# knights-lab/UTree

Hardware: AMD Instinct MI355X
Metric: reads classified/sec, 8 GB L2 CTR, 150 bp reads (higher is better)
Workload: dtype u64; 1 GPU; configs[1]: 1.22e+09-node synthetic L2 CTR (k=32, 21844 labels, image 40.8 GiB, fine_bits=8), 1152000000 x 150 bp reads per GPU (72 steps x 16000000-read batches, 41 distinct batches resident in HBM), RC=0

## Files before the change

utree_amd/csrc/dev_image.c:

```c
#define _FILE_OFFSET_BITS 64
#define _GNU_SOURCE
#define __HIP_PLATFORM_AMD__ 1
#include <hip/hip_runtime_api.h>
#include <fcntl.h>
#include <math.h>
#include <stddef.h>
#include <stdio.h>
#include <stdlib.h>
#include <string.h>
#include <unistd.h>
#include "ctr_host.h"
#include "dev_image.h"

#define HIPCHK(x) do { hipError_t e_ = (x); if (e_ != hipSuccess) { utree_dev_set_hip_error((int)e_, #x); rc = e_ == hipErrorOutOfMemory ? UTREE_E_NOMEM : UTREE_E_HIP; goto fail; } } while (0)
#define KCHK(x) do { int e_ = (x); if (e_ != 0) { utree_dev_set_hip_error(e_, #x); rc = e_ == (int)hipErrorOutOfMemory ? UTREE_E_NOMEM : UTREE_E_HIP; goto fail; } } while (0)

static __thread char g_hip_msg[256];
void utree_dev_set_hip_error(int err, const char *what) {
    snprintf(g_hip_msg, sizeof g_hip_msg, "%s (%d) in %s", hipGetErrorString((hipError_t)err), err, what);
    if (getenv("UTREE_DEBUG")) fprintf(stderr, "[utree_amd] HIP error: %s\n", g_hip_msg);
}
const char *utree_last_hip_error(void) { return g_hip_msg; }
void utree_set_error_text(const char *msg) { snprintf(g_hip_msg, sizeof g_hip_msg, "%s", msg); }

// ... 788 lines not shown
        d->last_long = w.long_blocks != 0; d->last_mid = 0; d->last_rc = do_rc; d->last_short_cap = w.short_cap;
        d->last_lanes = utk_lanes_segs(&d->kimg, max_len); d->last_mixed = mixed; d->last_pieces = w.long_blocks != 0;
        if (e0 && !w.long_blocks) HIPCHK(hipEventRecord(e0, st));
        if (!mixed) KCHK(utk_classify_lanes(&d->kimg, d_bases, d_off, d_len, n_reads, max_len, do_rc, d_out, &w, d->n_cu, st));
        else KCHK(utk_classify_lanes_mixed(&d->kimg, d_bases, d_off, d_len, n_reads, max_len, do_rc, d_out, &w, d->n_cu, st));
        if (w.long_blocks) {
            if (e0) HIPCHK(hipEventRecord(e0, st));
            HIPCHK(hipMemsetAsync(w.ltab_rank, 0xFF, (size_t)w.n_long_cap * UTREE_LONG_SLOTS * 4, st));
            HIPCHK(hipMemsetAsync(w.ltab_cnt, 0, (size_t)w.n_long_cap * UTREE_LONG_SLOTS * 4, st));
            HIPCHK(hipMemsetAsync(w.lflag, 0, (size_t)w.n_long_cap * 4, st));
            KCHK(utk_classify_long_pieces(&d->kimg, d_bases, d_off, d_len, do_rc, d_out, &w, d->n_cu, st));
            utk_workspace wl = w;
            wl.long_list = w.long_left;
            wl.long_blocks = w.long_blocks >= 8 ? w.long_blocks / 8 : 1;
            KCHK(utk_classify_long(&d->kimg, d_bases, d_off, d_len, do_rc, d_out, &wl, d->n_cu, st));
            if (e0) { HIPCHK(hipEventRecord(e1, st)); d->recorded[tslot] = 1; }
        }
        KCHK(utk_classify_listed(&d->kimg, d_bases, d_off, d_len, n_reads, max_len, do_rc, d_out, &w, d->n_cu, st));
        if (e0 && !w.long_blocks) { HIPCHK(hipEventRecord(e1, st)); d->recorded[tslot] = 1; }
    } else {
        const int dominant = w.long_blocks ? 2 : (w.mid_reads ? 1 : 0);
        d->last_long = dominant == 2; d->last_mid = dominant == 1; d->last_rc = do_rc; d->last_short_cap = w.short_cap;
        d->last_lanes = 0; d->last_mixed = 0; d->last_pieces = 0;
        if (w.mid_reads) KCHK(utk_route(d_len, n_reads, do_rc, &w, st));
        if (e0 && dominant == 0) HIPCHK(hipEventRecord(e0, st));
        KCHK(utk_classify_short(&d->kimg, d_bases, d_off, d_len, n_reads, do_rc, d_out, &w, d->n_cu, st));
        if (e0 && dominant == 0) { HIPCHK(hipEventRecord(e1, st)); d->recorded[tslot] = 1; }
        if (w.mid_reads) {
            if (e0 && dominant == 1) HIPCHK(hipEventRecord(e0, st));
            KCHK(utk_classify_mid(&d->kimg, d_bases, d_off, d_len, n_reads, do_rc, d_out, &w, d->n_cu, st));
            if (e0 && dominant == 1) { HIPCHK(hipEventRecord(e1, st)); d->recorded[tslot] = 1; }
        }
        if (w.long_blocks) {
            if (e0) HIPCHK(hipEventRecord(e0, st));
            KCHK(utk_classify_long(&d->kimg, d_bases, d_off, d_len, do_rc, d_out, &w, d->n_cu, st));
            if (e0) { HIPCHK(hipEventRecord(e1, st)); d->recorded[tslot] = 1; }
        }
    }
    if (rd && (rc = utree_redist_add_pending(rd, &d->kimg, d_out, &w, n_reads, d->n_cu, st))) goto fail;
    KCHK(utk_vote(&d->kimg, d_out, &w, n_reads, st));
    if (ring_post(d, &w, lanes ? n_reads : 0, st)) { (void)hipGetLastError(); }
    { ring_lock(d); const unsigned long long pe = d->dev_error; ring_unlock(d);
      if (pe) { rc = UTREE_E_DEVICE; snprintf(g_hip_msg, sizeof g_hip_msg, "an earlier batch's kernels reported error %llu: utree_classify_poll returns (and clears) it", pe); } }
#ifdef UTREE_LANES_TIMERS
    { extern void utk_lanes_phase_dump(void); static int lcalls; if (++lcalls == 6) utk_lanes_phase_dump(); }
#endif
#ifdef UTREE_PHASE_TIMERS
    { extern void utk_phase_dump(void); static int calls; if (++calls == 12) utk_phase_dump(); }
#endif
fail:
    return rc;
}

int utree_lookup_words(utree_dev *d, const uint64_t *d_hi, const uint64_t *d_lo, uint64_t n, uint32_t *d_ix, void *stream) {
    int rc = UTREE_OK;
    if (!d || !d_lo || !d_ix) return UTREE_E_ARG;
    if (d->hdr.W == 16 && !d_hi) return UTREE_E_ARG;
    HIPCHK(hipSetDevice(d->device));
    KCHK(utk_lookup(&d->kimg, d_hi, d_lo, n, d_ix, (hipStream_t)stream));
fail:
    return rc;
}

const char *utree_classify_kernel_name(const utree_dev *dc) {
    if (!dc) return "";
    utree_dev *d = (utree_dev *)dc;
    if (d->last_lanes && d->last_pieces) {
        snprintf(d->kernel_sig, sizeof d->kernel_sig, "classify_lanes_k<%u, %u, 16, %s, 2, %u, %s>", d->hdr.W, d->hdr.I, d->kimg.irr_n ? "true" : "false", d->hdr.bucket_words / 8,
                 utk_lanes_both_strands(&d->kimg, d->last_rc) ? "true" : "false");
        return d->kernel_sig;
    }
    if (d->last_lanes && d->last_mixed) {
        snprintf(d->kernel_sig, sizeof d->kernel_sig, "classify_lanes_mixed_k<%u, %u, %s, %u, %s>", d->hdr.W, d->hdr.I, d->kimg.irr_n ? "true" : "false",
                 d->hdr.bucket_words / 8, utk_lanes_both_strands(&d->kimg, d->last_rc) ? "true" : "false");
        return d->kernel_sig;
    }
    if (d->last_lanes) {
        snprintf(d->kernel_sig, sizeof d->kernel_sig, "classify_lanes_k<%u, %u, 1, %s, 0, %u, %s>", d->hdr.W, d->hdr.I, d->kimg.irr_n ? "true" : "false",
                 d->hdr.bucket_words / 8, utk_lanes_both_strands(&d->kimg, d->last_rc) ? "true" : "false");
        return d->kernel_sig;
    }
    return d->last_long ? utk_classify_long_name(&d->kimg, d->kernel_sig, sizeof d->kernel_sig)
                        : utk_classify_short_name(&d->kimg, d->last_short_cap ? d->last_short_cap : UTREE_SHORT_CAP, d->last_mid, d->last_rc,
                                                  d->kernel_sig, sizeof d->kernel_sig);
}

int utree_model_counts(utree_dev *d, const uint8_t *d_bases, const uint64_t *d_off, const uint32_t *d_len, uint32_t n_reads,
                       int do_rc, uint64_t *h_counts5, void *stream) {
    int rc = UTREE_OK;
    unsigned long long *dc = NULL;
    if (!d || !d_bases || !d_off || !d_len || !h_counts5) return UTREE_E_ARG;
    HIPCHK(hipSetDevice(d->device));
    HIPCHK(hipMalloc((void **)&dc, 64));
    HIPCHK(hipMemsetAsync(dc, 0, 64, (hipStream_t)stream));
    KCHK(utk_model_counts(&d->kimg, d_bases, d_off, d_len, n_reads, do_rc, dc, stream));
    HIPCHK(hipMemcpyAsync(h_counts5, dc, 40, hipMemcpyDeviceToHost, (hipStream_t)stream));
    HIPCHK(hipStreamSynchronize((hipStream_t)stream));
fail:
    if (dc) hipFree(dc);
    return rc;
}

int utree_classify_kernel_time(utree_dev *d, int reset, double *ms_total, uint64_t *launches) {
    int rc = UTREE_OK;
    if (!d) return UTREE_E_ARG;
    HIPCHK(hipSetDevice(d->device));
// ... 20 lines not shown
```

utree_amd/csrc/kernels.hip:

```cpp
#include <hip/hip_runtime.h>
#include <stdint.h>
#include <stdio.h>
#include <string.h>
#include "device_common.hpp"
#include "wave_common.hpp"

using namespace utk;

namespace {

#ifdef UTREE_PHASE_TIMERS
__device__ unsigned long long g_phase[16];
struct PhaseT { unsigned long long t, acc[12]; };
#define PH_DECL PhaseT ph_; ph_.t = __builtin_readcyclecounter(); for (int q_ = 0; q_ < 12; ++q_) ph_.acc[q_] = 0;
#define TICKP(ph, i) do { const unsigned long long n_ = __builtin_readcyclecounter(); (ph).acc[i] += n_ - (ph).t; (ph).t = n_; } while (0)
#define TICK(i) TICKP(ph_, i)
#define PH_ARG , PhaseT &ph_
#define PH_PASS , ph_
#define PH_WAITVM asm volatile("s_waitcnt vmcnt(0)" ::: "memory")
#else
#define PH_DECL
#define TICK(i)
#define PH_ARG
#define PH_PASS
// ... 618 lines not shown
__device__ __forceinline__ uint32_t cut_of(uint32_t x) {
    uint32_t c = x - x / 4;
    c += (x >> 1) >= c;
    return c;
}

__device__ __forceinline__ void label16(const char *s, uint32_t p, uint64_t &x, uint64_t &y) {
    typedef unsigned long long u64x2 __attribute__((ext_vector_type(2), aligned(1)));
    const u64x2 v = *(const u64x2 *)(s + p);
    x = v.x; y = v.y;
}

__device__ __forceinline__ uint64_t stop_flags(uint64_t x1, uint64_t x2) {
    const uint64_t semi = x1 ^ 0x3B3B3B3B3B3B3B3Bull, d = x1 ^ x2;
    uint64_t m = (((x1 - 0x0101010101010101ull) & ~x1) | ((semi - 0x0101010101010101ull) & ~semi)) & 0x8080808080808080ull;
    m |= (((d & 0x7F7F7F7F7F7F7F7Full) + 0x7F7F7F7F7F7F7F7Full) | d) & 0x8080808080808080ull;
    return m;
}

__device__ __forceinline__ void pair_scan(const char *s1, const char *s2, uint32_t start, uint32_t &td, uint32_t &a, uint32_t &b, uint32_t &before) {
    uint32_t base = start, prevlast = start ? (uint32_t)(uint8_t)s1[start - 1] : 0u;
    for (;;) {
        uint64_t x1, y1, x2, y2;
        label16(s1, base, x1, y1); label16(s2, base, x2, y2);
        uint64_t m = stop_flags(x1, x2);
        if (!m) { prevlast = (uint32_t)(x1 >> 56); base += 8; x1 = y1; x2 = y2; m = stop_flags(x1, x2); }
        if (m) {
            const uint32_t idx = (uint32_t)(__builtin_ctzll(m) >> 3);
            td = base + idx;
            a = (uint32_t)(x1 >> (8 * idx)) & 0xFFu; b = (uint32_t)(x2 >> (8 * idx)) & 0xFFu;
            before = idx ? ((uint32_t)(x1 >> (8 * idx - 8)) & 0xFFu) : prevlast;
            return;
        }
        prevlast = (uint32_t)(x1 >> 56); base += 8;
    }
}

struct VRec { uint64_t w[4]; };
__device__ __forceinline__ VRec vrec(const uint64_t *vt, uint32_t rank) {
    typedef unsigned long long u64x2 __attribute__((ext_vector_type(2)));
    const u64x2 *p = (const u64x2 *)(vt + (size_t)rank * 4);
    const u64x2 a = p[0], b = p[1];
    VRec v; v.w[0] = a.x; v.w[1] = a.y; v.w[2] = b.x; v.w[3] = b.y;
    return v;
}
__device__ __forceinline__ uint32_t v_pid(const VRec &v, uint32_t t) { return (uint32_t)((t < 4 ? v.w[0] : v.w[1]) >> (16u * (t & 3u))) & 0xFFFFu; }
__device__ __forceinline__ uint32_t v_end(const VRec &v, uint32_t t) { return (uint32_t)(v.w[2] >> (8u * t)) & 0xFFu; }
__device__ __forceinline__ bool v_exists(const VRec &v, uint32_t t) { return ((uint32_t)v.w[3] >> t) & 1u; }
__device__ __forceinline__ bool v_more(const VRec &v, uint32_t t) { return ((uint32_t)v.w[3] >> (8u + t)) & 1u; }
__device__ __forceinline__ bool v_us(const VRec &v, uint32_t t) { return ((uint32_t)v.w[3] >> (16u + t)) & 1u; }
__device__ __forceinline__ uint32_t v_len(const VRec &v) { return (uint32_t)(v.w[3] >> 32) & 0xFFu; }
__device__ __forceinline__ uint32_t v_ix(const VRec &v) { return (uint32_t)(v.w[3] >> 48); }

__device__ __forceinline__ void vote_table(const utk_image &im, utree_result *out_r, const uint64_t *T, uint32_t F, uint32_t uix) {
    const uint64_t *vt = im.vote_tab;
    const char *blob = im.label_blob;
    const uint32_t *loff = im.label_off;
    constexpr uint32_t NONE = 0xFFFFFFFFu;
    uint32_t cutoff = cut_of(F);
    uint32_t st = 0, ed = uix, dv = NONE, t = 0, orun = F, sl, ol;
    uint32_t ix_last, n_last, len_last;
    for (;;) {
        const uint64_t t_st = T[st];
        VRec pv = vrec(vt, (uint32_t)t_st);
        const uint64_t t_ed = ed - 1u == st ? t_st : T[ed - 1u];
        const VRec lv = ed - 1u == st ? pv : vrec(vt, (uint32_t)t_ed);
        {
            const uint64_t d0 = pv.w[0] ^ lv.w[0], d1 = pv.w[1] ^ lv.w[1];
            const uint32_t same = d0 ? (uint32_t)__builtin_ctzll(d0) >> 4 : 4u + (d1 ? (uint32_t)__builtin_ctzll(d1) >> 4 : 4u);
            const uint32_t both = ((uint32_t)(pv.w[3] & lv.w[3]) >> 8) & 0xFFu;
            const uint32_t semis = (uint32_t)__builtin_ctz(~both);
            const uint32_t L = same < semis ? same : semis;
            if (L > t) { dv = v_end(pv, L - 1u); t = L; }
        }
        uint32_t run = (uint32_t)(t_st >> 32), td = dv, c1 = run, rp = (uint32_t)t_st;
        bool td_is_end = false;
        bool stopped = false;
        for (uint32_t z = st + 1; z < ed; ++z) {
            const bool is_last = z == ed - 1u;
            const uint64_t tz = is_last ? t_ed : T[z];
            const uint32_t nz = (uint32_t)(tz >> 32), rc = (uint32_t)tz;
            const VRec cv = is_last ? lv : vrec(vt, rc);
            bool aside = false, stop = false;
            if (t >= 8u || !v_exists(pv, t) || (dv == NONE && v_end(pv, 0) == 0u && !v_more(pv, 0))) aside = true;
            else {
                uint32_t a, b, before;
                bool known = true;
                if (v_exists(cv, t) && v_pid(cv, t) == v_pid(pv, t)) {
                    td = v_end(pv, t); td_is_end = true;
                    a = v_more(pv, t) ? ';' : 0u; b = v_more(cv, t) ? ';' : 0u; before = v_us(pv, t) ? '_' : 'x';
                } else if (v_us(pv, t) || !v_exists(cv, t)) {
                    pair_scan(blob + loff[rp], blob + loff[rc], dv + 1u, td, a, b, before);
                    td_is_end = td == v_end(pv, t);
                } else { a = 'a'; b = 'b'; before = 'x'; known = false; }
                if (a == b) run += nz;
                else if ((!a && b == ';') || ((a == ';' || !a) && before == '_')) aside = true;
                else if (run >= cutoff) {
                    ed = z; stop = true;
                    if (!known) {
                        pair_scan(blob + loff[rp], blob + loff[rc], dv + 1u, td, a, b, before);
                        td_is_end = td == v_end(pv, t);
                    }
                } else { run = nz; st = z; }
            }
            if (aside) {
                run = nz; st = z;
                orun -= c1;
                cutoff = cut_of(orun);
            }
            if (stop) { stopped = true; break; }
            pv = cv; c1 = nz; rp = rc;
        }
        ix_last = stopped ? v_ix(pv) : v_ix(lv);
        n_last = stopped ? c1 : (uint32_t)(t_ed >> 32);
        len_last = stopped ? v_len(pv) : v_len(lv);
        sl = run; ol = orun;
        if (run < cutoff) break;
        if (st + 1 >= ed) {
            if (n_last >= cutoff) dv = 0xFFFFFFFEu;
            break;
        }
        orun = run; cutoff = cut_of(run);
        if (td != dv) { dv = td; if (td_is_end) ++t; }
    }
    int32_t cut;
    if (dv == NONE) cut = -1;
    else if (dv == 0xFFFFFFFEu) cut = -2;
    else cut = (int32_t)(dv < len_last ? dv : len_last);
    store_result(out_r, ix_last, cut, F, uix, sl, ol);
}

__global__ __launch_bounds__(256) void vote_table_k(utk_image im, utree_result *__restrict__ out, utk_workspace ws, uint32_t n_reads) {
    __shared__ uint32_t s_n[2][4];
    __shared__ uint16_t s_who[256];
    const uint32_t tid = threadIdx.x, wv = tid >> 6, lane = tid & 63u;
    const uint32_t r0 = blockIdx.x * blockDim.x + tid;
    uint32_t cls = 2;
    if (r0 < n_reads) {
        const uint32_t *res = (const uint32_t *)&out[r0];
        const int32_t cut = (int32_t)res[1];
        if (cut == RANK_PENDING) {
            uint32_t *o = (uint32_t *)&out[r0];
            o[0] = im.rank2ix[res[0]]; o[1] = (uint32_t)-2;
        } else if (cut == CUT_PENDING) cls = res[3] == 2u ? 0u : 1u;
    }
    const uint64_t m0 = __builtin_amdgcn_ballot_w64(cls == 0u), m1 = __builtin_amdgcn_ballot_w64(cls == 1u);
    s_who[tid] = 0xFFFFu;
    if (lane == 0) { s_n[0][wv] = (uint32_t)__popcll(m0); s_n[1][wv] = (uint32_t)__popcll(m1); }
    __syncthreads();
    if (cls < 2u) {
        uint32_t before = 0;
        for (uint32_t w = 0; w < wv; ++w) before += s_n[cls][w];
        before += (uint32_t)__popcll((cls ? m1 : m0) & ((1ull << lane) - 1ull));
        s_who[cls ? 255u - before : before] = (uint16_t)tid;
    }
    __syncthreads();
    const uint32_t who = s_who[tid];
    if (who == 0xFFFFu) return;
    const uint32_t r = blockIdx.x * blockDim.x + who;
    const uint32_t *res = (const uint32_t *)&out[r];
    vote_table(im, &out[r], ws.tally + ((uint64_t)res[4] | ((uint64_t)res[5] << 32)), res[2], res[3]);
}

__global__ __launch_bounds__(256) void vote_k(utk_image im, utree_result *__restrict__ out, utk_workspace ws, uint32_t n_reads) {
    const uint32_t r = blockIdx.x * blockDim.x + threadIdx.x;
    if (r >= n_reads) return;
    const uint32_t *res = (const uint32_t *)&out[r];
    if ((int32_t)res[1] == RANK_PENDING) {
        uint32_t *o = (uint32_t *)&out[r];
        o[0] = im.rank2ix[res[0]]; o[1] = (uint32_t)-2;
        return;
    }
    if ((int32_t)res[1] != CUT_PENDING) return;
    const uint32_t F = res[2], uix = res[3];
    const uint64_t *T = ws.tally + ((uint64_t)res[4] | ((uint64_t)res[5] << 32));
    const char *blob = im.label_blob;
    const uint32_t *loff = im.label_off;
    uint32_t cutoff = cut_of(F);
    uint32_t st = 0, ed = uix, dv = 0xFFFFFFFFu, orun = F, sl, ol;
    for (;;) {
        const uint64_t t_st = T[st];
        {
            const char *sa = blob + loff[(uint32_t)t_st], *sz = blob + loff[(uint32_t)T[ed - 1]];
            uint32_t base = dv + (dv == 0xFFFFFFFFu), q = 0xFFFFFFFFu;
            bool first = dv != 0xFFFFFFFFu;
            for (;;) {
                uint64_t a[2], b[2];
                label16(sa, base, a[0], a[1]); label16(sz, base, b[0], b[1]);
                bool stop = false;
#pragma unroll
                for (int h = 0; h < 2; ++h) {
                    const uint64_t x = a[h], d = a[h] ^ b[h], sx = a[h] ^ 0x3B3B3B3B3B3B3B3Bull;
                    uint64_t end = ((x - 0x0101010101010101ull) & ~x) & 0x8080808080808080ull;
                    end |= (((d & 0x7F7F7F7F7F7F7F7Full) + 0x7F7F7F7F7F7F7F7Full) | d) & 0x8080808080808080ull;
                    uint64_t semi = ~(((sx & 0x7F7F7F7F7F7F7F7Full) + 0x7F7F7F7F7F7F7F7Full) | sx) & 0x8080808080808080ull;
                    if (h == 0 && first) { end &= ~0xFFull; semi &= ~0xFFull; }
                    if (end) semi &= (end & (0ull - end)) - 1ull;
                    if (semi) q = base + 8u * (uint32_t)h + ((63u - (uint32_t)__builtin_clzll(semi)) >> 3);
                    if (end) { stop = true; break; }
                }
                if (stop) break;
                base += 16; first = false;
            }
            if (q != 0xFFFFFFFFu) dv = q;
        }
        uint32_t run = (uint32_t)(t_st >> 32), td = dv;
        const char *s1 = blob + loff[(uint32_t)t_st];
        uint32_t c1 = run;
        const uint32_t probe = dv + (dv == 0xFFFFFFFFu);
        const bool skip0 = dv != 0xFFFFFFFFu;
        uint64_t x1_first, y1_first;
        label16(s1, probe, x1_first, y1_first);
        for (uint32_t z = st + 1; z < ed; ++z) {
            const uint64_t tz = T[z];
// ... 146 lines not shown
    });
}

int utk_route(const uint32_t *d_len, uint32_t n_reads, int do_rc, const utk_workspace *ws, void *stream) {
    if (!n_reads) return 0;
    route_k<<<dim3((n_reads + 255) / 256), dim3(256), 0, (hipStream_t)stream>>>(d_len, n_reads, do_rc, *ws);
    return (int)hipGetLastError();
}

int utk_classify_mid(const utk_image *im, const uint8_t *d_bases, const uint64_t *d_off, const uint32_t *d_len,
                     uint32_t n_reads, int do_rc, utree_result *d_out, const utk_workspace *ws, int n_cu, void *stream) {
    if (!n_reads) return 0;
    uint32_t blocks = (n_reads + WAVES_PER_BLOCK - 1) / WAVES_PER_BLOCK;
    uint32_t cap = (uint32_t)n_cu * 5u;
    if (blocks > cap) blocks = cap;
    return dispatch_img_all(im, [&](auto w, auto i, auto exc, auto offt) {
        classify_short_k<decltype(w)::value, decltype(i)::value, decltype(exc)::value, decltype(offt), MID_CAP, true>
            <<<dim3(blocks), dim3(256), 0, (hipStream_t)stream>>>(*im, d_bases, d_off, d_len, n_reads, do_rc, d_out, *ws);
    });
}

int utk_classify_listed(const utk_image *im, const uint8_t *d_bases, const uint64_t *d_off, const uint32_t *d_len,
                        uint32_t n_reads, uint32_t max_len, int do_rc, utree_result *d_out, const utk_workspace *ws, int n_cu, void *stream) {
    if (!n_reads) return 0;
    uint32_t blocks = (n_reads + WAVES_PER_BLOCK - 1) / WAVES_PER_BLOCK;
    uint32_t cap = (uint32_t)n_cu * 2u;
    if (blocks > cap) blocks = cap;
    const uint64_t total = do_rc ? 2ull * max_len + 1 : max_len;
    return dispatch_img(im, [&](auto w, auto i, auto exc, auto offt) {
        if (total > SHORT2_CAP)
            classify_short_k<decltype(w)::value, decltype(i)::value, decltype(exc)::value, decltype(offt), MID_CAP, true>
                <<<dim3(blocks), dim3(256), 0, (hipStream_t)stream>>>(*im, d_bases, d_off, d_len, n_reads, do_rc, d_out, *ws);
        else if (do_rc || total > SHORT_CAP)
            classify_short_k<decltype(w)::value, decltype(i)::value, decltype(exc)::value, decltype(offt), SHORT2_CAP, true>
                <<<dim3(blocks), dim3(256), 0, (hipStream_t)stream>>>(*im, d_bases, d_off, d_len, n_reads, do_rc, d_out, *ws);
        else
            classify_short_k<decltype(w)::value, decltype(i)::value, decltype(exc)::value, decltype(offt), SHORT_CAP, true, 0>
                <<<dim3(blocks), dim3(256), 0, (hipStream_t)stream>>>(*im, d_bases, d_off, d_len, n_reads, do_rc, d_out, *ws);
    });
}

int utk_classify_long(const utk_image *im, const uint8_t *d_bases, const uint64_t *d_off, const uint32_t *d_len,
                      int do_rc, utree_result *d_out, const utk_workspace *ws, int n_cu, void *stream) {
    (void)n_cu;
    if (!ws->long_blocks) return 0;
    return dispatch_img_all(im, [&](auto w, auto i, auto exc, auto offt) {
        classify_long_k<decltype(w)::value, decltype(i)::value, decltype(exc)::value, decltype(offt)>
            <<<dim3(ws->long_blocks), dim3(LONG_THREADS), 0, (hipStream_t)stream>>>(*im, d_bases, d_off, d_len, do_rc, d_out, *ws);
    });
}

int utk_vote(const utk_image *im, utree_result *d_out, const utk_workspace *ws, uint32_t n_reads, void *stream) {
    if (!n_reads) return 0;
    if (im->vote_tab) vote_table_k<<<dim3((n_reads + 255) / 256), dim3(256), 0, (hipStream_t)stream>>>(*im, d_out, *ws, n_reads);
    else vote_k<<<dim3((n_reads + 255) / 256), dim3(256), 0, (hipStream_t)stream>>>(*im, d_out, *ws, n_reads);
    return (int)hipGetLastError();
}

int utk_lookup(const utk_image *im, const uint64_t *d_hi, const uint64_t *d_lo, uint64_t n, uint32_t *d_ix, void *stream) {
    if (!n) return 0;
    uint64_t blocks = (n + 255) / 256;
    if (blocks > 8192) blocks = 8192;
    return dispatch_img_all(im, [&](auto w, auto i, auto exc, auto offt) {
        lookup_k<decltype(w)::value, decltype(i)::value, decltype(exc)::value, decltype(offt)>
            <<<dim3((unsigned)blocks), dim3(256), 0, (hipStream_t)stream>>>(*im, d_hi, d_lo, n, d_ix);
    });
}

#ifdef UTREE_PHASE_TIMERS
void utk_phase_dump(void) {
    unsigned long long h[16];
    static const char *nm[12] = {"grab", "next read's len/off + fetch issue", "minimizers", "round: address (LDS chain) + load issue", "round: wait for the bucket",
                                 "round: scan", "round: hit compaction", "stage next read (waits for its bytes)", "tally + result", "after windows", "", ""};
    if (hipDeviceSynchronize() != hipSuccess || hipMemcpyFromSymbol(h, HIP_SYMBOL(g_phase), sizeof h) != hipSuccess) return;
    unsigned long long tot = 0;
    for (int q = 0; q < 12; ++q) tot += h[q];
    fprintf(stderr, "[phase timers] %llu waves, %.3g cycles per wave\n", h[12], h[12] ? (double)tot / h[12] : 0.0);
    for (int q = 0; q < 10; ++q) fprintf(stderr, "  %-45s %5.1f %%\n", nm[q], tot ? 100.0 * h[q] / tot : 0.0);
    memset(h, 0, sizeof h);
    (void)hipMemcpyToSymbol(HIP_SYMBOL(g_phase), h, sizeof h);
}
#endif

int utk_model_counts(const utk_image *im, const uint8_t *d_bases, const uint64_t *d_off, const uint32_t *d_len, uint32_t n_reads,
                     int do_rc, unsigned long long *d_counts, void *stream) {
    if (!n_reads) return 0;
    uint32_t blocks = (n_reads + 3) / 4;
    if (blocks > 4096) blocks = 4096;
    return dispatch_wi(im->W, im->I, [&](auto w, auto i) {
        model_k<decltype(w)::value, decltype(i)::value><<<dim3(blocks), dim3(256), 0, (hipStream_t)stream>>>(*im, d_bases, d_off, d_len, n_reads,
                                                                                                      do_rc, d_counts);
    });
}

static const char *kernel_signature(char *buf, size_t cap, const char *name, const utk_image *im, int slice, int listed, int rcmode) {
    const bool exc = (im->flags & (UTREE_F_IRREGULAR | UTREE_F_GENERIC)) != 0, o64 = (im->flags & UTREE_F_OFF64) != 0;
    if (slice) snprintf(buf, cap, "%s<%u, %u, %s, %s, %d, %s, %d>", name, im->W, im->I, exc ? "true" : "false", o64 ? "unsigned long" : "unsigned int",
                        slice, listed ? "true" : "false", rcmode);
    else snprintf(buf, cap, "%s<%u, %u, %s, %s>", name, im->W, im->I, exc ? "true" : "false", o64 ? "unsigned long" : "unsigned int");
    return buf;
}
const char *utk_classify_short_name(const utk_image *im, uint32_t short_cap, int mid, int do_rc, char *buf, size_t cap) {
    if (mid) return kernel_signature(buf, cap, "classify_short_k", im, MID_CAP, 1, 2);
    if (short_cap == UTREE_SHORT2_CAP) return kernel_signature(buf, cap, "classify_short_k", im, SHORT2_CAP, 0, 2);
    return kernel_signature(buf, cap, "classify_short_k", im, SHORT_CAP, 0, do_rc ? 1 : 0);
}
const char *utk_classify_long_name(const utk_image *im, char *buf, size_t cap) { return kernel_signature(buf, cap, "classify_long_k", im, 0, 0, 0); }
// ... 3 lines not shown
```

utree_amd/csrc/utree_internal.h:

```cpp
#ifndef UTREE_INTERNAL_H
#define UTREE_INTERNAL_H
#include <stddef.h>
#include <stdint.h>
#include <stdlib.h>
#include <time.h>
#include "../../include/utree_amd.h"

#ifdef __cplusplus
extern "C" {
#endif

#define UTREE_NUMBINS ((1u << 24) + 1u)
#define UTREE_INVALID 0xFFFFFFFFu
#define UTREE_IMG_MAGIC 0x31474d4945525455ull
#define UTREE_IMG_HEADER_BYTES 4096u
#define UTREE_IMG_VERSION 14u
#define UTREE_REGION_NB_BITS 25
#define UTREE_REGION_SUB_BITS 9
#define UTREE_REGION_BASE_SHIFT (UTREE_REGION_NB_BITS + UTREE_REGION_SUB_BITS)
#define UTREE_MIN_MARGIN(W_) ((W_) == 16 ? 2u : 0u)
#define UTREE_TALLY_CHUNK 8192u
#define UTREE_CUR_LONG 32
#define UTREE_CUR_MID 16
#define UTREE_CUR_WORK 48
// ... 78 lines not shown
                  const uint64_t *d_regions, const uint64_t *h_regions, uint64_t n_buckets, uint32_t bucket_words, uint64_t *d_table, uint64_t *d_mrecs,
                  uint32_t *d_irreg, unsigned long long *d_overflow, uint64_t *n_min, int *views, void *stream);
int utk_build_direct(uint32_t I, int off64, int generic, const void *d_coarse, const uint64_t *d_recs, uint64_t n_nodes, uint64_t c0, uint64_t m,
                     const uint32_t *d_irreg, uint64_t n_irregular, void *d_table, void *stream);
int utk_compact_overflow(uint32_t W, uint32_t I, uint64_t *d_table, uint64_t n_buckets, uint32_t bucket_words, uint64_t *d_mrecs, uint64_t *n_kept, int *chains, void *stream);
int utk_compress_chunk(uint32_t W, uint32_t I, const void *d_in, uint64_t first, uint64_t count, unsigned long long *d_first,
                       void *d_out, void *stream);
int utk_fill_recs_pad(uint64_t *d_recs_end, uint32_t words, void *stream);

typedef struct {
    unsigned long long *cursors;
    uint64_t *tally;
    uint64_t tally_cap;
    uint32_t *long_list;
    uint32_t *mid_list;
    uint32_t *hist;
    uint32_t *touch;
    uint32_t long_blocks, mid_reads;
    uint32_t short_cap;
    uint32_t mid_limit;
    uint64_t *pieces;
    uint32_t *ltab_rank, *ltab_cnt;
    uint32_t *lflag;
    uint32_t *long_left;
    uint32_t n_long_cap;
    uint64_t n_pieces_cap;
    uint32_t *cls_list;
    uint32_t cls_stride;
    uint64_t ltally_base;
} utk_workspace;

int utk_classify_short(const utk_image *im, const uint8_t *d_bases, const uint64_t *d_off, const uint32_t *d_len,
                       uint32_t n_reads, int do_rc, utree_result *d_out, const utk_workspace *ws, int n_cu,
                       void *stream);
int utk_lanes_ok(const utk_image *im, uint32_t max_len, int do_rc);
int utk_lanes_segs(const utk_image *im, uint32_t max_len);
int utk_lanes_image_ok(const utk_image *im);
int utk_lanes_both_strands(const utk_image *im, int do_rc);
int utk_classify_long_pieces(const utk_image *im, const uint8_t *d_bases, const uint64_t *d_off, const uint32_t *d_len, int do_rc,
                             utree_result *d_out, const utk_workspace *ws, int n_cu, void *stream);
int utk_classify_lanes(const utk_image *im, const uint8_t *d_bases, const uint64_t *d_off, const uint32_t *d_len, uint32_t n_reads,
                       uint32_t max_len, int do_rc, utree_result *d_out, const utk_workspace *ws, int n_cu, void *stream);
int utk_classify_lanes_mixed(const utk_image *im, const uint8_t *d_bases, const uint64_t *d_off, const uint32_t *d_len, uint32_t n_reads,
                             uint32_t max_len, int do_rc, utree_result *d_out, const utk_workspace *ws, int n_cu, void *stream);
uint32_t utk_lanes_max_len(const utk_image *im);
int utk_route(const uint32_t *d_len, uint32_t n_reads, int do_rc, const utk_workspace *ws, void *stream);
int utk_classify_mid(const utk_image *im, const uint8_t *d_bases, const uint64_t *d_off, const uint32_t *d_len,
                     uint32_t n_reads, int do_rc, utree_result *d_out, const utk_workspace *ws, int n_cu, void *stream);
int utk_classify_listed(const utk_image *im, const uint8_t *d_bases, const uint64_t *d_off, const uint32_t *d_len,
                        uint32_t n_reads, uint32_t max_len, int do_rc, utree_result *d_out, const utk_workspace *ws, int n_cu, void *stream);
int utk_classify_long(const utk_image *im, const uint8_t *d_bases, const uint64_t *d_off, const uint32_t *d_len,
                      int do_rc, utree_result *d_out, const utk_workspace *ws, int n_cu, void *stream);
int utk_vote(const utk_image *im, utree_result *d_out, const utk_workspace *ws, uint32_t n_reads, void *stream);
int utk_lookup(const utk_image *im, const uint64_t *d_hi, const uint64_t *d_lo, uint64_t n, uint32_t *d_ix,
               void *stream);
typedef struct {
    unsigned long long *cursors;
    uint32_t *nh;
    uint64_t *hoff;
    uint32_t *hits;
    uint64_t hits_cap;
    uint32_t *lvl[3];
    uint32_t nlvl[3];
    uint32_t *hist;
    uint32_t hist_waves;
    uint32_t *state;
    uint32_t state_cap;
    uint32_t step;
    uint32_t slack, tolerance;
} utk_rank_ws;

int utk_rank_hits(const utk_image *im, const uint8_t *d_bases, const uint64_t *d_off, const uint32_t *d_len,
                  uint32_t n_reads, int do_rc, const utk_rank_ws *ws, int n_cu, void *stream);
int utk_rank_levels(const utk_rank_ws *ws, uint32_t n_reads, void *stream);
int utk_rank_vote(const utk_image *im, utree_result *d_out, uint32_t n_reads, const utk_rank_ws *ws, int n_cu,
                  void *stream);
int utk_rank_state(uint32_t n_reads, const utk_rank_ws *ws, void *stream);

const char *utk_classify_short_name(const utk_image *im, uint32_t short_cap, int mid, int do_rc, char *buf, size_t cap);
const char *utk_classify_long_name(const utk_image *im, char *buf, size_t cap);
int utk_model_counts(const utk_image *im, const uint8_t *d_bases, const uint64_t *d_off, const uint32_t *d_len, uint32_t n_reads,
                     int do_rc, unsigned long long *d_counts, void *stream);

static inline double now_s(void) { struct timespec ts; clock_gettime(CLOCK_MONOTONIC, &ts); return (double)ts.tv_sec + 1e-9 * (double)ts.tv_nsec; }
static inline int timing_on(void) { return getenv("UTREE_TIMING") != NULL || getenv("UTREE_DEBUG") != NULL; }
int utree_pread_team(int fd, void *dst, size_t bytes, uint64_t off, int max_threads);

#ifdef __cplusplus
}
#endif
#endif
```

utree_amd/lib.py:

```python
from __future__ import annotations

import ctypes as C
import os

_HERE = os.path.dirname(os.path.abspath(__file__))
SO_PATH = os.environ.get("UTREE_AMD_SO") or os.path.join(_HERE, "libutree_amd.so")
CLI_PATH = os.path.join(_HERE, "xtree-searchGG")
COMPRESS_CLI_PATH = os.path.join(_HERE, "xtree-compress")
RANK_CLI_PATH = os.path.join(_HERE, "xtree-search")
BUILD_GG_CLI_PATH = os.path.join(_HERE, "utree-buildGG")
BUILD_CLI_PATH = os.path.join(_HERE, "utree-build")
_LIB = None

OK, E_IO, E_FORMAT, E_UNSUPPORTED, E_NOMEM, E_HIP, E_ARG, E_NOLABELS, E_FASTA, E_RCCL, E_BUILD, E_DEVICE, E_PROFILE, E_COVERAGE, E_PAIRS = range(15)
BUILD_E_MAP_EMPTY, BUILD_E_MAP, BUILD_E_FASTA, BUILD_E_NO_KMERS, BUILD_E_NAME = range(1, 6)
FINE_AUTO = -1
FANOUT_NONE, FANOUT_BROADCAST, FANOUT_UPLOAD = range(3)
REPLICATE_FN = C.CFUNCTYPE(C.c_int, C.c_void_p, C.c_void_p, C.POINTER(C.c_int), C.c_int, C.POINTER(C.c_void_p))
UPLOAD_FN = C.CFUNCTYPE(C.c_int, C.c_void_p, C.c_int, C.c_int, C.POINTER(C.c_void_p))
INPUT_REFERENCE, INPUT_FASTQ, INPUT_FASTA_MULTILINE, INPUT_AUTO = range(4)


class CtrInfo(C.Structure):
    _fields_ = [("W", C.c_uint32), ("I", C.c_uint32), ("k", C.c_uint32), ("SZ", C.c_uint32), ("n_nodes", C.c_uint64),
# ... 112 lines not shown
    "utree_rank_search_file": (C.c_int, [C.c_void_p, C.c_void_p, C.c_char_p, C.c_char_p, C.c_int, C.POINTER(RankParams),
                                         C.c_int, C.POINTER(SearchStats)]),
    "utree_reads_frame": (C.c_int, [C.c_void_p, C.c_size_t, C.c_int, C.c_int, C.c_size_t, C.c_void_p, C.c_void_p, C.c_void_p,
                                    C.c_void_p, C.POINTER(C.c_size_t), C.POINTER(C.c_size_t), C.POINTER(FastaError)]),
    "utree_search_file_opts": (C.c_int, [C.c_void_p, C.POINTER(C.c_void_p), C.c_int, C.c_char_p, C.c_char_p, C.c_int, C.c_int,
                                         C.c_int, C.POINTER(SearchStats)]),
    "utree_rank_search_file_opts": (C.c_int, [C.c_void_p, C.c_void_p, C.c_char_p, C.c_char_p, C.c_int, C.POINTER(RankParams),
                                              C.c_int, C.c_int, C.POINTER(SearchStats)]),
    "utree_build_file": (C.c_int, [C.c_char_p, C.c_char_p, C.c_char_p, C.c_uint32, C.c_uint32, C.c_int, C.c_int, C.c_int,
                                   C.POINTER(BuildStats)]),
    "utree_search_prepare": (C.c_int, [C.c_void_p, C.POINTER(C.c_void_p), C.c_int, C.c_int]),
    "utree_search_file": (C.c_int, [C.c_void_p, C.POINTER(C.c_void_p), C.c_int, C.c_char_p, C.c_char_p, C.c_int, C.c_int,
                                    C.POINTER(SearchStats)]),
    "utree_profile_create": (C.c_int, [C.c_void_p, C.c_uint32, C.POINTER(C.c_void_p)]),
    "utree_profile_add": (C.c_int, [C.c_void_p, C.c_void_p, C.c_uint32, C.c_void_p]),
    "utree_profile_reset": (C.c_int, [C.c_void_p]),
    "utree_profile_max_entries": (C.c_size_t, [C.c_void_p]),
    "utree_profile_read": (C.c_int, [C.c_void_p, C.c_void_p, C.c_size_t, C.POINTER(C.c_size_t), C.POINTER(C.c_uint64),
                                     C.POINTER(C.c_uint64)]),
    "utree_profile_free": (None, [C.c_void_p]),
    "utree_profile_write": (C.c_int, [C.c_void_p, C.c_void_p, C.c_size_t, C.c_uint64, C.c_char_p]),
    "utree_search_file_profile": (C.c_int, [C.c_void_p, C.POINTER(C.c_void_p), C.c_int, C.c_char_p, C.c_char_p, C.c_int, C.c_int,
                                            C.c_int, C.c_char_p, C.POINTER(SearchStats)]),
    "utree_coverage_bytes": (C.c_size_t, [C.c_void_p]),
    "utree_coverage_create": (C.c_int, [C.c_void_p, C.c_void_p, C.c_void_p, C.c_void_p, C.POINTER(C.c_void_p)]),
    "utree_coverage_add": (C.c_int, [C.c_void_p, C.c_void_p, C.c_void_p, C.c_void_p, C.c_uint32, C.c_int, C.c_void_p]),
    "utree_coverage_reset": (C.c_int, [C.c_void_p]),
    "utree_coverage_merge": (C.c_int, [C.c_void_p, C.c_void_p]),
    "utree_coverage_read": (C.c_int, [C.c_void_p, C.c_void_p, C.c_size_t, C.POINTER(C.c_size_t), C.POINTER(C.c_uint64),
                                      C.POINTER(C.c_uint64)]),
    "utree_coverage_free": (None, [C.c_void_p]),
    "utree_coverage_write": (C.c_int, [C.c_void_p, C.c_void_p, C.c_size_t, C.c_uint64, C.c_char_p]),
    "utree_search_file_coverage": (C.c_int, [C.c_void_p, C.POINTER(C.c_void_p), C.c_int, C.c_char_p, C.c_char_p, C.c_int, C.c_int,
                                             C.c_int, C.c_char_p, C.c_char_p, C.POINTER(SearchStats)]),
    "utree_redist_create": (C.c_int, [C.c_void_p, C.c_uint32, C.POINTER(C.c_void_p)]),
    "utree_redist_reset": (C.c_int, [C.c_void_p]),
    "utree_redist_free": (None, [C.c_void_p]),
    "utree_redist_classify_batch": (C.c_int, [C.c_void_p, C.c_void_p, C.c_void_p, C.c_void_p, C.c_void_p, C.c_uint32, C.c_uint64,
                                              C.c_uint32, C.c_int, C.c_void_p, C.c_void_p, C.c_size_t, C.c_void_p]),
    "utree_redist_read": (C.c_int, [C.c_void_p, C.c_void_p, C.c_size_t, C.c_void_p, C.c_size_t, C.POINTER(C.c_size_t), C.POINTER(C.c_size_t),
                                    C.POINTER(C.c_uint64), C.POINTER(C.c_uint64)]),
    "utree_redist_merge": (C.c_int, [C.c_void_p, C.c_void_p]),
    "utree_redist_solve": (C.c_int, [C.c_void_p, C.c_uint32, C.c_void_p, C.c_size_t, C.POINTER(C.c_size_t), C.POINTER(C.c_uint32),
                                     C.POINTER(C.c_uint64)]),
    "utree_redist_write": (C.c_int, [C.c_void_p, C.c_void_p, C.c_size_t, C.c_uint64, C.c_uint64, C.c_uint32, C.c_char_p]),
    "utree_search_file_redistribute": (C.c_int, [C.c_void_p, C.POINTER(C.c_void_p), C.c_int, C.c_char_p, C.c_char_p, C.c_int, C.c_char_p, C.c_int,
                                                 C.c_int, C.c_int, C.c_char_p, C.c_char_p, C.c_char_p, C.c_uint32, C.POINTER(SearchStats)]),
    "utree_pairs_join": (C.c_int, [C.c_void_p, C.c_void_p, C.c_void_p, C.c_void_p, C.c_void_p, C.c_void_p, C.c_void_p, C.c_uint32, C.c_void_p,
                                   C.c_uint64, C.c_void_p, C.c_void_p, C.c_void_p, C.c_void_p]),
    "utree_search_pairs_file": (C.c_int, [C.c_void_p, C.POINTER(C.c_void_p), C.c_int, C.c_char_p, C.c_char_p, C.c_char_p, C.c_int, C.c_int,
                                          C.c_int, C.c_char_p, C.c_char_p, C.POINTER(SearchStats)]),
    "utree_rank_search_file_profile": (C.c_int, [C.c_void_p, C.c_void_p, C.c_char_p, C.c_char_p, C.c_int, C.POINTER(RankParams),
                                                 C.c_int, C.c_int, C.c_char_p, C.POINTER(SearchStats)]),
}


def kernel_source_sha256() -> str:
    import hashlib
    h = hashlib.sha256()
    for f in ("kernels.hip", "lanes_kernel.hip", "lanes_core.hpp", "lanes_part.hip", "wave_common.hpp", "device_common.hpp", "utree_internal.h", "Makefile"):
        with open(os.path.join(_HERE, "csrc", f), "rb") as fh:
            h.update(f.encode() + b"\0" + fh.read() + b"\0")
    return h.hexdigest()


class UtreeError(RuntimeError):
    def __init__(self, code, what=""):
        self.code = code
        msg = load().utree_strerror(code).decode() if _LIB is not None else str(code)
        if _LIB is not None and code in (4, 5, 11, 12, 13, 14):
            hip = (_LIB.utree_last_hip_error() or b"").decode(errors="replace")
            if hip:
                msg += " [" + hip + "]"
        super().__init__("%s: %s (code %d)" % (what, msg, code))


def load():
    global _LIB
    if _LIB is None:
        if not os.path.exists(SO_PATH):
            raise ImportError("utree_amd: %s is missing -- build it with `make -C utree_amd/csrc` "
                              "(or __graft_entry__.build()); there is no CPU fallback" % SO_PATH)
        try:
            import torch
        except ImportError:
            pass
        L = C.CDLL(SO_PATH, mode=C.RTLD_GLOBAL)
        for name, (res, args) in SYMBOLS.items():
            f = getattr(L, name)
            f.restype = res
            f.argtypes = args
        _LIB = L
    return _LIB


def check(code, what=""):
    if code != OK:
        raise UtreeError(code, what)
```

Before: 2.358 billion reads/s.

## Bin vote-table reads by label count per 2048-read tile and specialize small cases

The vote_table kernel now processes 2048-read tiles per block. It classifies pending reads into buckets by distinct-label count (2, 3, 4, other), compacts them through shared memory so each wavefront runs reads of the same size class, and calls vote_table instances templated on N with the loop unrolled and, for two labels, records preloaded. The aim is to cut wavefront divergence and loop overhead in the LCA vote. It also adds a host-side utree_vote_lists test entry point, which is unrelated to speed. The risks are more shared-memory and register pressure and fewer blocks in flight.

```diff
diff --git a/utree_amd/csrc/dev_image.c b/utree_amd/csrc/dev_image.c
--- a/utree_amd/csrc/dev_image.c
+++ b/utree_amd/csrc/dev_image.c
@@ -864,6 +864,65 @@
     return rc;
 }
 
+static int vote_ent_cmp(const void *a, const void *b) {
+    const uint64_t x = *(const uint64_t *)a, y = *(const uint64_t *)b;
+    return (uint32_t)x < (uint32_t)y ? -1 : (uint32_t)x > (uint32_t)y;
+}
+int utree_vote_lists(utree_dev *d, const uint32_t *h_ix, const uint32_t *h_cnt, const uint32_t *h_first, uint32_t n_reads, utree_result *h_out) {
+    int rc = UTREE_OK;
+    if (!d || !h_first || !h_out || (h_first[n_reads] && (!h_ix || !h_cnt))) return UTREE_E_ARG;
+    if (!n_reads) return UTREE_OK;
+    const uint32_t n_labels = d->hdr.n_labels, total = h_first[n_reads];
+    uint32_t *ix2rank = (uint32_t *)calloc((size_t)n_labels + 1, 4), *r2i = (uint32_t *)malloc(((size_t)n_labels + 1) * 4);
+    uint64_t *tally = (uint64_t *)malloc(((size_t)total + 1) * 8);
+    uint32_t *rec = (uint32_t *)calloc((size_t)n_reads, sizeof(utree_result));
+    void *d_out = NULL, *d_tally = NULL;
+    if (!ix2rank || !r2i || !tally || !rec) { rc = UTREE_E_NOMEM; goto fail; }
+    HIPCHK(hipSetDevice(d->device));
+    HIPCHK(hipMemcpy(r2i, d->kimg.rank2ix, (size_t)n_labels * 4, hipMemcpyDeviceToHost));
+    for (uint32_t r = 0; r < n_labels; ++r) if (r2i[r] < n_labels) ix2rank[r2i[r]] = r;
+    uint64_t used = 0;
+    for (uint32_t r = 0; r < n_reads; ++r) {
+        if (h_first[r + 1] < h_first[r] || h_first[r + 1] > total) { rc = UTREE_E_ARG; goto fail; }
+        uint64_t *T = tally + used;
+        uint32_t nu = 0, F = 0;
+        for (uint32_t j = h_first[r]; j < h_first[r + 1]; ++j) {
+            if (h_ix[j] >= n_labels) { rc = UTREE_E_ARG; goto fail; }
+            if (!h_cnt[j]) continue;
+            T[nu++] = (uint64_t)ix2rank[h_ix[j]] | ((uint64_t)h_cnt[j] << 32);
+            F += h_cnt[j];
+        }
+        qsort(T, nu, 8, vote_ent_cmp);
+        uint32_t m = 0;
+        for (uint32_t j = 0; j < nu; ++j) {
+            if (m && (uint32_t)T[m - 1] == (uint32_t)T[j]) T[m - 1] += T[j] & 0xFFFFFFFF00000000ull;
+            else T[m++] = T[j];
+        }
+        uint32_t *o = rec + (size_t)r * 6;
+        o[2] = F; o[3] = m;
+        if (m == 0) o[1] = (uint32_t)-2;
+        else if (m == 1) { o[0] = (uint32_t)T[0]; o[1] = (uint32_t)-4; }
+        else { o[1] = (uint32_t)-3; o[4] = (uint32_t)used; o[5] = (uint32_t)(used >> 32); used += m; }
+    }
+    HIPCHK(hipMalloc(&d_out, (size_t)n_reads * sizeof(utree_result)));
+    HIPCHK(hipMalloc(&d_tally, ((size_t)used + 1) * 8));
+    HIPCHK(hipMemcpy(d_out, rec, (size_t)n_reads * sizeof(utree_result), hipMemcpyHostToDevice));
+    HIPCHK(hipMemcpy(d_tally, tally, (size_t)used * 8, hipMemcpyHostToDevice));
+    {
+        utk_workspace w;
+        memset(&w, 0, sizeof w);
+        w.tally = (uint64_t *)d_tally; w.tally_cap = used;
+        KCHK(utk_vote(&d->kimg, (utree_result *)d_out, &w, n_reads, NULL));
+    }
+    HIPCHK(hipDeviceSynchronize());
+    HIPCHK(hipMemcpy(h_out, d_out, (size_t)n_reads * sizeof(utree_result), hipMemcpyDeviceToHost));
+fail:
+    if (d_out) (void)hipFree(d_out);
+    if (d_tally) (void)hipFree(d_tally);
+    free(ix2rank); free(r2i); free(tally); free(rec);
+    return rc;
+}
+
 int utree_lookup_words(utree_dev *d, const uint64_t *d_hi, const uint64_t *d_lo, uint64_t n, uint32_t *d_ix, void *stream) {
     int rc = UTREE_OK;
     if (!d || !d_lo || !d_ix) return UTREE_E_ARG;
diff --git a/utree_amd/csrc/kernels.hip b/utree_amd/csrc/kernels.hip
--- a/utree_amd/csrc/kernels.hip
+++ b/utree_amd/csrc/kernels.hip
@@ -694,7 +694,9 @@
 __device__ __forceinline__ uint32_t v_len(const VRec &v) { return (uint32_t)(v.w[3] >> 32) & 0xFFu; }
 __device__ __forceinline__ uint32_t v_ix(const VRec &v) { return (uint32_t)(v.w[3] >> 48); }
 
-__device__ __forceinline__ void vote_table(const utk_image &im, utree_result *out_r, const uint64_t *T, uint32_t F, uint32_t uix) {
+template <uint32_t N>
+__device__ __forceinline__ void vote_table(const utk_image &im, utree_result *out_r, const uint64_t *T, uint32_t F, uint32_t uix_arg) {
+    const uint32_t uix = N ? N : uix_arg;
     const uint64_t *vt = im.vote_tab;
     const char *blob = im.label_blob;
     const uint32_t *loff = im.label_off;
@@ -702,11 +704,15 @@
     uint32_t cutoff = cut_of(F);
     uint32_t st = 0, ed = uix, dv = NONE, t = 0, orun = F, sl, ol;
     uint32_t ix_last, n_last, len_last;
+    uint64_t t_two[2] = {0, 0};
+    VRec r_two[2] = {};
+    if (N == 2) { t_two[0] = T[0]; t_two[1] = T[1]; r_two[0] = vrec(vt, (uint32_t)t_two[0]); r_two[1] = vrec(vt, (uint32_t)t_two[1]); }
     for (;;) {
-        const uint64_t t_st = T[st];
-        VRec pv = vrec(vt, (uint32_t)t_st);
-        const uint64_t t_ed = ed - 1u == st ? t_st : T[ed - 1u];
-        const VRec lv = ed - 1u == st ? pv : vrec(vt, (uint32_t)t_ed);
+        if (N == 2) { st = 0; ed = 2; }
+        const uint64_t t_st = N == 2 ? t_two[0] : T[st];
+        VRec pv = N == 2 ? r_two[0] : vrec(vt, (uint32_t)t_st);
+        const uint64_t t_ed = N == 2 ? t_two[1] : (ed - 1u == st ? t_st : T[ed - 1u]);
+        const VRec lv = N == 2 ? r_two[1] : (ed - 1u == st ? pv : vrec(vt, (uint32_t)t_ed));
         {
             const uint64_t d0 = pv.w[0] ^ lv.w[0], d1 = pv.w[1] ^ lv.w[1];
             const uint32_t same = d0 ? (uint32_t)__builtin_ctzll(d0) >> 4 : 4u + (d1 ? (uint32_t)__builtin_ctzll(d1) >> 4 : 4u);
@@ -718,7 +724,7 @@
         uint32_t run = (uint32_t)(t_st >> 32), td = dv, c1 = run, rp = (uint32_t)t_st;
         bool td_is_end = false;
         bool stopped = false;
-        for (uint32_t z = st + 1; z < ed; ++z) {
+        auto pair = [&](const uint32_t z) -> bool {
             const bool is_last = z == ed - 1u;
             const uint64_t tz = is_last ? t_ed : T[z];
             const uint32_t nz = (uint32_t)(tz >> 32), rc = (uint32_t)tz;
@@ -750,8 +756,16 @@
                 orun -= c1;
                 cutoff = cut_of(orun);
             }
-            if (stop) { stopped = true; break; }
+            if (stop) { stopped = true; return true; }
             pv = cv; c1 = nz; rp = rc;
+            return false;
+        };
+        if (N == 0) {
+            for (uint32_t z = st + 1; z < ed; ++z) if (pair(z)) break;
+        } else {
+            const uint32_t z0 = st + 1u;
+#pragma unroll
+            for (uint32_t k = 0; k + 1u < N; ++k) { if (z0 + k >= ed) break; if (pair(z0 + k)) break; }
         }
         ix_last = stopped ? v_ix(pv) : v_ix(lv);
         n_last = stopped ? c1 : (uint32_t)(t_ed >> 32);
@@ -772,36 +786,75 @@
     store_result(out_r, ix_last, cut, F, uix, sl, ol);
 }
 
+constexpr uint32_t VT_TILE = 2048, VT_PER = VT_TILE / 256;
 __global__ __launch_bounds__(256) void vote_table_k(utk_image im, utree_result *__restrict__ out, utk_workspace ws, uint32_t n_reads) {
-    __shared__ uint32_t s_n[2][4];
-    __shared__ uint16_t s_who[256];
-    const uint32_t tid = threadIdx.x, wv = tid >> 6, lane = tid & 63u;
-    const uint32_t r0 = blockIdx.x * blockDim.x + tid;
-    uint32_t cls = 2;
-    if (r0 < n_reads) {
-        const uint32_t *res = (const uint32_t *)&out[r0];
-        const int32_t cut = (int32_t)res[1];
-        if (cut == RANK_PENDING) {
-            uint32_t *o = (uint32_t *)&out[r0];
-            o[0] = im.rank2ix[res[0]]; o[1] = (uint32_t)-2;
-        } else if (cut == CUT_PENDING) cls = res[3] == 2u ? 0u : 1u;
-    }
-    const uint64_t m0 = __builtin_amdgcn_ballot_w64(cls == 0u), m1 = __builtin_amdgcn_ballot_w64(cls == 1u);
-    s_who[tid] = 0xFFFFu;
-    if (lane == 0) { s_n[0][wv] = (uint32_t)__popcll(m0); s_n[1][wv] = (uint32_t)__popcll(m1); }
+    __shared__ uint16_t s_pos[VT_TILE];
+    __shared__ uint32_t s_cnt[4][4];
+    const uint32_t tid = threadIdx.x, wv = (uint32_t)__builtin_amdgcn_readfirstlane((int)(tid >> 6));
+    const uint64_t tile0 = (uint64_t)blockIdx.x * VT_TILE;
+    uint32_t w0[VT_PER], w1[VT_PER], w3[VT_PER];
+#pragma unroll
+    for (uint32_t i = 0; i < VT_PER; ++i) {
+        const uint64_t r = tile0 + i * 256u + tid;
+        const uint32_t *res = (const uint32_t *)&out[r < n_reads ? r : n_reads - 1u];
+        w0[i] = res[0]; w1[i] = r < n_reads ? res[1] : 0u; w3[i] = res[3];
+    }
+    uint32_t cls = 0, cnt[4] = {0, 0, 0, 0};
+#pragma unroll
+    for (uint32_t i = 0; i < VT_PER; ++i) {
+        uint32_t c = 7u;
+        if ((int32_t)w1[i] == RANK_PENDING) {
+            uint32_t *o = (uint32_t *)&out[tile0 + i * 256u + tid];
+            o[0] = im.rank2ix[w0[i]]; o[1] = (uint32_t)-2;
+        } else if ((int32_t)w1[i] == CUT_PENDING) c = w3[i] - 2u < 3u ? w3[i] - 2u : 3u;
+        cls |= c << (3u * i);
+#pragma unroll
+        for (uint32_t k = 0; k < 4; ++k) cnt[k] += (uint32_t)__popcll(__builtin_amdgcn_ballot_w64(c == k));
+    }
+    if ((tid & 63u) == 0) {
+#pragma unroll
+        for (uint32_t k = 0; k < 4; ++k) s_cnt[k][wv] = cnt[k];
+    }
     __syncthreads();
-    if (cls < 2u) {
-        uint32_t before = 0;
-        for (uint32_t w = 0; w < wv; ++w) before += s_n[cls][w];
-        before += (uint32_t)__popcll((cls ? m1 : m0) & ((1ull << lane) - 1ull));
-        s_who[cls ? 255u - before : before] = (uint16_t)tid;
+    uint32_t n[4], at[4], first[4];
+    {
+        uint32_t sum = 0;
+#pragma unroll
+        for (int k = 3; k >= 0; --k) {
+            first[k] = sum;
+            uint32_t mine = sum;
+#pragma unroll
+            for (uint32_t w = 0; w < 4; ++w) { const uint32_t v = s_cnt[k][w]; if (w < wv) mine += v; sum += v; }
+            n[k] = (uint32_t)__builtin_amdgcn_readfirstlane((int)(sum - first[k]));
+            at[k] = (uint32_t)__builtin_amdgcn_readfirstlane((int)mine);
+            first[k] = (uint32_t)__builtin_amdgcn_readfirstlane((int)first[k]);
+        }
+    }
+#pragma unroll
+    for (uint32_t i = 0; i < VT_PER; ++i) {
+        const uint32_t c = (cls >> (3u * i)) & 7u;
+#pragma unroll
+        for (uint32_t k = 0; k < 4; ++k) {
+            const uint64_t m = __builtin_amdgcn_ballot_w64(c == k);
+            if (c == k) s_pos[at[k] + __builtin_amdgcn_mbcnt_hi((uint32_t)(m >> 32), __builtin_amdgcn_mbcnt_lo((uint32_t)m, 0u))] = (uint16_t)(i * 256u + tid);
+            at[k] += (uint32_t)__popcll(m);
+        }
     }
     __syncthreads();
-    const uint32_t who = s_who[tid];
-    if (who == 0xFFFFu) return;
-    const uint32_t r = blockIdx.x * blockDim.x + who;
-    const uint32_t *res = (const uint32_t *)&out[r];
-    vote_table(im, &out[r], ws.tally + ((uint64_t)res[4] | ((uint64_t)res[5] << 32)), res[2], res[3]);
+    const uint32_t ns3 = (n[3] + 63u) >> 6, ns2 = (n[2] + 63u) >> 6, ns1 = (n[1] + 63u) >> 6, ns0 = (n[0] + 63u) >> 6;
+    for (uint32_t s = wv; s < ns3 + ns2 + ns1 + ns0; s += 4) {
+        uint32_t q = s, k = 3;
+        if (q >= ns3) { q -= ns3; k = 2; if (q >= ns2) { q -= ns2; k = 1; if (q >= ns1) { q -= ns1; k = 0; } } }
+        const uint32_t e = q * 64u + (tid & 63u);
+        if (e >= n[k]) continue;
+        const uint64_t r = tile0 + s_pos[first[k] + e];
+        const uint32_t *res = (const uint32_t *)&out[r];
+        const uint64_t *T = ws.tally + ((uint64_t)res[4] | ((uint64_t)res[5] << 32));
+        if (k == 0) vote_table<2>(im, &out[r], T, res[2], 2);
+        else if (k == 1) vote_table<3>(im, &out[r], T, res[2], 3);
+        else if (k == 2) vote_table<4>(im, &out[r], T, res[2], 4);
+        else vote_table<0>(im, &out[r], T, res[2], res[3]);
+    }
 }
 
 __global__ __launch_bounds__(256) void vote_k(utk_image im, utree_result *__restrict__ out, utk_workspace ws, uint32_t n_reads) {
@@ -1054,7 +1107,7 @@
 
 int utk_vote(const utk_image *im, utree_result *d_out, const utk_workspace *ws, uint32_t n_reads, void *stream) {
     if (!n_reads) return 0;
-    if (im->vote_tab) vote_table_k<<<dim3((n_reads + 255) / 256), dim3(256), 0, (hipStream_t)stream>>>(*im, d_out, *ws, n_reads);
+    if (im->vote_tab) vote_table_k<<<dim3((unsigned)(((uint64_t)n_reads + VT_TILE - 1) / VT_TILE)), dim3(256), 0, (hipStream_t)stream>>>(*im, d_out, *ws, n_reads);
     else vote_k<<<dim3((n_reads + 255) / 256), dim3(256), 0, (hipStream_t)stream>>>(*im, d_out, *ws, n_reads);
     return (int)hipGetLastError();
 }
diff --git a/utree_amd/csrc/utree_internal.h b/utree_amd/csrc/utree_internal.h
--- a/utree_amd/csrc/utree_internal.h
+++ b/utree_amd/csrc/utree_internal.h
@@ -154,6 +154,8 @@
 int utk_classify_long(const utk_image *im, const uint8_t *d_bases, const uint64_t *d_off, const uint32_t *d_len,
                       int do_rc, utree_result *d_out, const utk_workspace *ws, int n_cu, void *stream);
 int utk_vote(const utk_image *im, utree_result *d_out, const utk_workspace *ws, uint32_t n_reads, void *stream);
+struct utree_dev;
+int utree_vote_lists(struct utree_dev *dev, const uint32_t *h_ix, const uint32_t *h_cnt, const uint32_t *h_first, uint32_t n_reads, utree_result *h_out);
 int utk_lookup(const utk_image *im, const uint64_t *d_hi, const uint64_t *d_lo, uint64_t n, uint32_t *d_ix,
                void *stream);
 typedef struct {
diff --git a/utree_amd/lib.py b/utree_amd/lib.py
--- a/utree_amd/lib.py
+++ b/utree_amd/lib.py
@@ -188,6 +188,7 @@
                                           C.c_int, C.c_char_p, C.c_char_p, C.POINTER(SearchStats)]),
     "utree_rank_search_file_profile": (C.c_int, [C.c_void_p, C.c_void_p, C.c_char_p, C.c_char_p, C.c_int, C.POINTER(RankParams),
                                                  C.c_int, C.c_int, C.c_char_p, C.POINTER(SearchStats)]),
+    "utree_vote_lists": (C.c_int, [C.c_void_p, C.c_void_p, C.c_void_p, C.c_void_p, C.c_uint32, C.c_void_p]),
 }
 
 
```

Result: slower. 2.277 billion reads/s (-3.4%).
